# Christovis/astrild

Hardware: AMD Instinct MI355X
Metric: particles/sec CIC+3D-FFT P(k) on 1024^3 grid (higher is better)
Workload: dtype f32

## Files before the change

### astrild_amd/csrc/fft_tile.hip

```cpp
#include "ast_common.h"
#include "paint_tile_geom.h"
#include <algorithm>
#include <cmath>
#include <cstring>
#include <mutex>
#include <vector>

namespace {

__device__ constexpr float kCos32[16] = {
    1.0f, 0.9807852804032304f, 0.9238795325112867f, 0.8314696123025452f, 0.7071067811865476f,
    0.5555702330196023f, 0.38268343236508984f, 0.19509032201612833f, 0.0f, -0.1950903220161282f,
    -0.3826834323650897f, -0.555570233019602f, -0.7071067811865475f, -0.8314696123025453f,
    -0.9238795325112867f, -0.9807852804032304f};
__device__ constexpr float kSin32[16] = {
    0.0f, 0.19509032201612825f, 0.3826834323650898f, 0.5555702330196022f, 0.7071067811865475f,
    0.8314696123025452f, 0.9238795325112867f, 0.9807852804032304f, 1.0f, 0.9807852804032304f,
    0.9238795325112867f, 0.8314696123025455f, 0.7071067811865476f, 0.5555702330196022f,
    0.3826834323650899f, 0.1950903220161286f};

#ifndef FFT_NT
#define FFT_NT 3
#endif
typedef float f2v __attribute__((ext_vector_type(2)));
template <bool NT>
__device__ inline float2 ld_stream(const float2* p) {
    if (NT && (FFT_NT & 1)) { const f2v v = __builtin_nontemporal_load(reinterpret_cast<const f2v*>(p)); return make_float2(v.x, v.y); }
    return *p;
}
template <bool NT>
__device__ inline void st_stream(float2* p, float2 v) {
    if (NT && (FFT_NT & 2)) __builtin_nontemporal_store(f2v{v.x, v.y}, reinterpret_cast<f2v*>(p));
    else *p = v;
}
typedef float cf2 __attribute__((ext_vector_type(2)));
__device__ inline cf2 to_cf(float2 a) { return cf2{a.x, a.y}; }
__device__ inline float2 from_cf(cf2 a) { return make_float2(a.x, a.y); }
__device__ inline cf2 cmul_cf(cf2 a, cf2 w) {
    return __builtin_elementwise_fma(a.yy, cf2{-w.y, w.x}, a.xx * w);
}
__device__ inline float2 cmul(float2 a, float2 w) { return from_cf(cmul_cf(to_cf(a), to_cf(w))); }

constexpr int bitrev(int v, int bits) {
    int r = 0;
    for (int i = 0; i < bits; ++i) r |= ((v >> i) & 1) << (bits - 1 - i);
    return r;
}
constexpr int ilog2(int v) { return v <= 1 ? 0 : 1 + ilog2(v / 2); }

template <int R>
__device__ inline void fft_reg(float2 (&vv)[R]) {
    cf2 v[R];
#pragma unroll
    for (int i = 0; i < R; ++i) v[i] = to_cf(vv[i]);
#pragma unroll
    for (int h = R / 2; h >= 1; h /= 2) {
#pragma unroll
        for (int blk = 0; blk < R; blk += 2 * h) {
#pragma unroll
            for (int j = 0; j < h; ++j) {
                const cf2 a = v[blk + j], b = v[blk + j + h];
                v[blk + j] = a + b;
                const cf2 d = a - b;
                const int t = j * (16 / h);
                if (t == 0) v[blk + j + h] = d;
                else if (t == 8) v[blk + j + h] = d.yx * cf2{1.0f, -1.0f};
                else v[blk + j + h] = cmul_cf(d, cf2{kCos32[t], -kSin32[t]});
            }
        }
    }
#pragma unroll
    for (int i = 0; i < R; ++i) vv[i] = from_cf(v[i]);
}

__device__ inline int tile_isqrt(int v) {
    return (int)__builtin_amdgcn_sqrtf((float)v + 0.5f);
}

__global__ void tile_isqrt_table_kernel(int* out, int count) {
    for (int v = blockIdx.x * blockDim.x + threadIdx.x; v < count; v += gridDim.x * blockDim.x) out[v] = tile_isqrt(v);
}

struct ShellMask { const float2* src; long long lo2, hi2; int ky0 = 0; int pass = 0;
                   size_t src_elem_stride = 0, src_batch_stride = 0; };

constexpr int SHELL_BATCH = 8;
#ifndef C2C_XCD_MODE
#define C2C_XCD_MODE 2
#endif
struct ShellBatch { int count = 0; float2* work[SHELL_BATCH]; long long lo2[SHELL_BATCH], hi2[SHELL_BATCH]; };
struct C2RBatch { int count = 0; const float2* in[SHELL_BATCH]; float* out[SHELL_BATCH]; int kmax[SHELL_BATCH]; };

struct DiscEntry { int offb; unsigned S, cumS, lohi; };
struct PackDst { float2* out = nullptr; unsigned c1_log2 = 0; unsigned nbatch = 0; float2* self_out = nullptr; unsigned self_part = ~0u; unsigned pitch = 0;
                 const DiscEntry* disc = nullptr; const unsigned short* gk = nullptr; unsigned part = 0;
                 unsigned xmajor = 0; };

template <int R1, int R2, int C, bool POWER, bool INV = false, int PACK = 0>
__global__ void __launch_bounds__(C * (R1 > R2 ? R1 : R2))
__attribute__((amdgpu_waves_per_eu((POWER || C > 16) && R1 * R2 >= 1024 ? 4 : 1, (POWER || C > 16) && R1 * R2 >= 1024 ? 4 : 8)))
strided_c2c_kernel(float2* __restrict__ data, const float2* __restrict__ tw_g, size_t elem_stride,
                   size_t ncols, size_t batch_stride, unsigned tiles_per_batch, float scale,
                   double* __restrict__ partial, const unsigned* __restrict__ edge_fall, ShellMask mask = ShellMask{nullptr, 0, 0},
                   PackDst pack = PackDst{}, ShellBatch sb = ShellBatch{}) {
    constexpr int N = R1 * R2;
    constexpr int NT = C * (R1 > R2 ? R1 : R2);
    constexpr int NB = N / 2 - 1;
    constexpr bool SPLIT = (POWER || C > 16) && R1 == R2 && N * C * sizeof(float2) > 64 * 1024;
    constexpr int YN = SPLIT ? N / 2 : N;
    extern __shared__ float2 lds[];
    float2* Y = lds;
    float2* tw = lds + YN * C;
    double* shell = reinterpret_cast<double*>(lds + YN * C + N);
    unsigned tile = blockIdx.x % tiles_per_batch, b = blockIdx.x / tiles_per_batch;
#if C2C_XCD_MODE
    if ((INV || C2C_XCD_MODE == 2) && (gridDim.x / tiles_per_batch) % 8u == 0u) {
        const unsigned xcd = blockIdx.x & 7u, slot = blockIdx.x >> 3;
        b = (slot / tiles_per_batch) * 8u + xcd;
        tile = slot % tiles_per_batch;
    }
#endif
    const size_t c0 = (size_t)tile * C;
    if (INV && sb.count > 0) {
        data = sb.work[blockIdx.y];
        mask.lo2 = sb.lo2[blockIdx.y];
        mask.hi2 = sb.hi2[blockIdx.y];
    }
    if (INV && mask.hi2 > 0) {
        const long long kb = (long long)((int)b > N / 2 ? (int)b - N : (int)b);
        const long long r2 = (long long)(c0 * c0) + (mask.pass == 0 ? kb * kb : 0);
        if (r2 >= mask.hi2) return;
    }
    const float2* disc_base = nullptr;
    unsigned disc_S = 0;
    int disc_ky = 0;
    if (!INV && POWER && pack.disc != nullptr) {
        const unsigned subb = b % R1, gk = pack.gk[pack.part * (pack.nbatch / R1) + b / R1];
        const DiscEntry e = pack.disc[(size_t)tile * R2 + gk];
        const unsigned lo = e.lohi & 255u, hi = (e.lohi >> 8) & 255u;
        if (subb - lo >= hi - lo) {
            for (int i = threadIdx.x; i < NB; i += NT) partial[((size_t)b * tiles_per_batch + tile) * NB + i] = 0.0;
            return;
        }
        disc_ky = (int)(gk * R1 + subb);
        if (pack.xmajor) {
            disc_base = data + ((long long)e.offb + (long long)(subb * 16u)) * (long long)pack.xmajor;
            disc_S = 16u;
        } else {
            disc_base = data + ((long long)e.offb + (long long)(subb * 16u));
            disc_S = e.S;
        }
    } else if (!INV && POWER && mask.hi2 > 0) {
        const long long kyi = (long long)b + mask.ky0, ky = kyi > N / 2 ? kyi - N : kyi;
        if (ky * ky + (long long)(c0 * c0) > mask.hi2) {
            for (int i = threadIdx.x; i < NB; i += NT) partial[((size_t)b * tiles_per_batch + tile) * NB + i] = 0.0;
            return;
        }
    }
    for (int i = threadIdx.x; i < N; i += NT) tw[i] = tw_g[i];
    if (POWER)
        for (int i = threadIdx.x; i <= NB; i += NT) shell[i] = 0.0;
    const int c = threadIdx.x % C, sub = threadIdx.x / C;
    const bool col_ok = (unsigned)c0 + (unsigned)c < (unsigned)ncols;
    float2 u[R2];
    {
        const bool task1 = sub < R2;
        float2 v[R1];
        const bool own = INV && mask.src != nullptr && mask.src_elem_stride != 0;
        size_t es_in = own ? mask.src_elem_stride : elem_stride;
        const float2* ubase = (INV && mask.src ? mask.src : data) + (size_t)b * (own ? mask.src_batch_stride : batch_stride);
        const int lsub = task1 ? sub : R2 - 1;
        uint32_t voff = (uint32_t)lsub * (uint32_t)es_in + min((uint32_t)c0 + (uint32_t)c, (uint32_t)ncols - 1u);
        if (POWER && !INV && disc_base != nullptr) {
            es_in = disc_S;
            ubase = disc_base;
            voff = (uint32_t)lsub * disc_S + (uint32_t)c;
        }
        if (INV && mask.hi2 > 0 && mask.pass == 1) {
            const long long c02 = (long long)(c0 * c0);
#pragma unroll
            for (int n1 = 0; n1 < R1; ++n1) {
                const int row = n1 * R2 + lsub;
                const long long ky = row > N / 2 ? row - N : row;
                v[n1] = make_float2(0.f, 0.f);
                if (ky * ky + c02 < mask.hi2) v[n1] = (ubase + (size_t)(n1 * R2) * es_in)[voff];
            }
        } else if (INV && mask.hi2 > 0) {
            const long long kyb = (long long)((int)b > N / 2 ? (int)b - N : (int)b);
            const long long r2yz = kyb * kyb + (long long)(c0 * c0);
#pragma unroll
            for (int n1 = 0; n1 < R1; ++n1) {
                const int lo = n1 * R2, hi = lo + R2 - 1;
                const long long kxmin = hi <= N / 2 ? lo : (lo >= N / 2 ? N - hi : 0);
                v[n1] = make_float2(0.f, 0.f);
                if (kxmin * kxmin + r2yz < mask.hi2) v[n1] = (ubase + (size_t)(n1 * R2) * es_in)[voff];
            }
        } else {
#pragma unroll
            for (int n1 = 0; n1 < R1; ++n1) v[n1] = ld_stream<(!INV && N >= 1024)>(ubase + (size_t)(n1 * R2) * es_in + voff);
        }
        if (INV) {
            if (mask.hi2 > 0 && mask.pass == 0) {
                const long long kz = (long long)min(c0 + c, ncols - 1), ky = (long long)((int)b > N / 2 ? (int)b - N : (int)b);
                const long long m2yz = ky * ky + kz * kz;
#pragma unroll
                for (int n1 = 0; n1 < R1; ++n1) {
                    const int row = n1 * R2 + lsub;
                    const long long kx = row > N / 2 ? row - N : row, m2 = kx * kx + m2yz;
                    if (m2 < mask.lo2 || m2 >= mask.hi2) v[n1] = make_float2(0.f, 0.f);
                }
            }
#pragma unroll
            for (int n1 = 0; n1 < R1; ++n1) v[n1].y = -v[n1].y;
        }
        fft_reg<R1>(v);
        __syncthreads();
        if (!SPLIT) {
            if (task1) {
#pragma unroll
                for (int k1 = 0; k1 < R1; ++k1) {
                    float2 y = v[bitrev(k1, ilog2(R1))];
                    if (k1 != 0) y = cmul(y, tw[sub * k1]);
                    Y[(sub * R1 + k1) * C + c] = y;
                }
            }
            __syncthreads();
            if (sub < R1) {
#pragma unroll
                for (int n2 = 0; n2 < R2; ++n2) u[n2] = Y[(n2 * R1 + sub) * C + c];
            }
        } else {
            constexpr int H = R2 / 2;
#pragma unroll
            for (int half = 0; half < 2; ++half) {
                if (sub / H == half) {
#pragma unroll
                    for (int k1 = 0; k1 < R1; ++k1) {
                        float2 y = v[bitrev(k1, ilog2(R1))];
                        if (k1 != 0) y = cmul(y, tw[sub * k1]);
                        Y[((sub - half * H) * R1 + k1) * C + c] = y;
                    }
                }
                __syncthreads();
#pragma unroll
                for (int nh = 0; nh < H; ++nh) u[half * H + nh] = Y[(nh * R1 + sub) * C + c];
                if (half == 0) __syncthreads();
            }
        }
    }
    if (sub < R1) {
        fft_reg<R2>(u);
        int tid_s = (int)threadIdx.x;
        if (C > 16) asm volatile("" : "+v"(tid_s));
        const int cs = C > 16 ? tid_s % C : c;
        const bool ok_s = C > 16 ? (unsigned)c0 + (unsigned)cs < (unsigned)ncols : col_ok;
        if (PACK == 2 && !POWER) {
            static_assert(PACK != 2 || C == 16, "the disc layout's tiles are 16 columns");
            const int4 ev = reinterpret_cast<const int4*>(pack.disc + (size_t)tile * R2)[threadIdx.x % R2];
#pragma unroll
            for (int k2 = 0; k2 < R2; ++k2) {
                float2 x = u[bitrev(k2, ilog2(R2))];
                x.x *= scale;
                x.y *= scale;
                const int offb = __builtin_amdgcn_readlane(ev.x, k2);
                const unsigned S = (unsigned)__builtin_amdgcn_readlane(ev.y, k2), cumS = (unsigned)__builtin_amdgcn_readlane(ev.z, k2);
                const unsigned lohi = (unsigned)__builtin_amdgcn_readlane(ev.w, k2);
                const unsigned lo = lohi & 255u, hi = (lohi >> 8) & 255u, part = lohi >> 16;
                if (pack.xmajor) {
                    float2* const ub = pack.self_out + ((long long)offb * (long long)pack.xmajor + (long long)(b * 16u));
                    if ((unsigned)sub - lo < hi - lo)
                        st_stream<(N >= 1024)>(ub + ((uint32_t)sub * 16u * pack.xmajor + (uint32_t)(threadIdx.x & 15u)), x);
                    continue;
                }
                float2* const ub = (part == pack.self_part ? pack.self_out : pack.out + (size_t)pack.nbatch * cumS)
                                   + ((size_t)b * S + (long long)offb);
                if ((unsigned)sub - lo < hi - lo) st_stream<(N >= 1024)>(ub + threadIdx.x, x);
            }
        } else if (ok_s && !POWER) {
            float2* const base = data + (size_t)b * batch_stride + c0 + cs;
            const int room = (!INV && mask.hi2 > 0) ? (int)mask.hi2 - (int)(c0 * c0) : 0x7fffffff;
            const int wsub0 = __builtin_amdgcn_readfirstlane((int)threadIdx.x) / C, wsub1 = wsub0 + 64 / C - 1;
#pragma unroll
            for (int k2 = 0; k2 < R2; ++k2) {
                float2 x = u[bitrev(k2, ilog2(R2))];
                x.x *= scale;
                x.y *= INV ? -scale : scale;
                if (!INV) {
                    const int aky = R1 * k2 >= N / 2 ? N - (wsub1 + R1 * k2) : wsub0 + R1 * k2;
                    if (aky * aky > room) continue;
                }
                if (PACK) {
                    const unsigned part = (unsigned)(R1 * k2) >> pack.c1_log2, r0 = (unsigned)(R1 * k2) & ((1u << pack.c1_log2) - 1u);
                    float2* const ub = part == pack.self_part
                        ? pack.self_out + ((((size_t)b) << pack.c1_log2) + r0) * pack.pitch
                        : pack.out + ((((size_t)part * pack.nbatch + b) << pack.c1_log2) + r0) * pack.pitch;
                    st_stream<(N >= 1024)>(ub + ((uint32_t)sub * pack.pitch + (uint32_t)c0 + (uint32_t)cs), x);
                } else {
                    st_stream<(!INV && N >= 1024)>(base + (size_t)(sub + R1 * k2) * elem_stride, x);
                }
            }
        }
    }
    int tid_e = (int)threadIdx.x;
    asm volatile("" : "+v"(tid_e));
    if (POWER && (unsigned)c0 + (unsigned)(tid_e % C) < (unsigned)ncols && sub < R1) {
        unsigned fallmask = 0;
        const int kyi = disc_base != nullptr ? disc_ky : (int)b + mask.ky0;
        if (edge_fall) fallmask = edge_fall[((size_t)(disc_base != nullptr ? (unsigned)disc_ky : b) * tiles_per_batch + tile) * NT + threadIdx.x];
        const int kz = (int)c0 + tid_e % C;
        const int ky = kyi > N / 2 ? kyi - N : kyi;
        const int m2yz = ky * ky + kz * kz;
        const float w = (kz > 0 && kz < N / 2) ? 2.0f : 1.0f;
#pragma unroll
        for (int k2 = 0; k2 < R2; ++k2) {
            const float2 x = u[bitrev(k2, ilog2(R2))];
            const int row = sub + R1 * k2;
            const int kx = row > N / 2 ? row - N : row;
            int sh = tile_isqrt(kx * kx + m2yz);
            sh -= (int)((fallmask >> k2) & 1u);
            if (sh >= 1 && sh <= NB) atomicAdd(&shell[sh], (double)(fmaf(x.x, x.x, x.y * x.y) * w));
        }
    }
    if (POWER) {
        __syncthreads();
        const double s2 = (double)scale * (double)scale;
        for (int i = threadIdx.x; i < NB; i += NT) partial[((size_t)b * tiles_per_batch + tile) * NB + i] = shell[i + 1] * s2;
    }
}

constexpr int REDUCE_ROWS = 1024;
__global__ void __launch_bounds__(256)
shell_partials_stage1_kernel(const double* __restrict__ partial, size_t nwg, int nb, double* __restrict__ partial2) {
    const size_t per = (nwg + REDUCE_ROWS - 1) / REDUCE_ROWS;
    const size_t g0 = (size_t)blockIdx.x * per, g1 = g0 + per < nwg ? g0 + per : nwg;
    for (int bin = threadIdx.x; bin < nb; bin += 256) {
        double acc = 0.0;
#pragma unroll 8
        for (size_t g = g0; g < g1; ++g) acc += partial[g * nb + bin];
        partial2[(size_t)blockIdx.x * nb + bin] = acc;
    }
}
__global__ void __launch_bounds__(256)
shell_partials_stage2_kernel(const double* __restrict__ partial2, int nb, double pnorm, int first_bin,
                             double* __restrict__ psum) {
    __shared__ double part[32][8];
    const int b8 = threadIdx.x & 7, grp = threadIdx.x >> 3;
    const int bin = blockIdx.x * 8 + b8;
    double acc = 0.0;
    if (bin < nb) {
#pragma unroll 8
        for (int r = grp; r < REDUCE_ROWS; r += 32) acc += partial2[(size_t)r * nb + bin];
    }
    part[grp][b8] = acc;
    __syncthreads();
    if (grp == 0 && bin < nb && bin >= first_bin) {
        double t = 0.0;
        for (int k = 0; k < 32; ++k) t += part[k][b8];
        psum[bin] += pnorm * t;
    }
}

constexpr int MLOW_FWD = 5, MBOX_FWD = MLOW_FWD + 1;
__device__ constexpr double kC16f[16] = {1.0, 0.92387953251128674, 0.70710678118654752, 0.38268343236508977, 0.0,
                                         -0.38268343236508977, -0.70710678118654752, -0.92387953251128674, -1.0,
                                         -0.92387953251128674, -0.70710678118654752, -0.38268343236508977, 0.0,
                                         0.38268343236508977, 0.70710678118654752, 0.92387953251128674};
__device__ constexpr double kS16f[16] = {0.0, -0.38268343236508977, -0.70710678118654752, -0.92387953251128674, -1.0,
                                         -0.92387953251128674, -0.70710678118654752, -0.38268343236508977, 0.0,
                                         0.38268343236508977, 0.70710678118654752, 0.92387953251128674, 1.0,
                                         0.92387953251128674, 0.70710678118654752, 0.38268343236508977};

struct SlabFold { int xb0 = 0, ntx = 0, row_lo = 0, row_hi = 0; bool ranges = false; };

template <int R1, int R2, int C, int FOLDW, bool LOWK = false>
__global__ void __launch_bounds__(C * R2)
__attribute__((amdgpu_waves_per_eu(LOWK ? 4 : 1, LOWK ? 4 : 8)))
rows_r2c_kernel(const float* __restrict__ in, float2* __restrict__ out, const float2* __restrict__ tw_g,
                size_t nrows, size_t in_pitch, size_t out_pitch, float scale, float mean,
                const float* __restrict__ rec, const double2* __restrict__ lowk_lane = nullptr,
                double* __restrict__ lowz = nullptr, SlabFold sf = SlabFold{}) {
    constexpr int M = R1 * R2, N = 2 * M;
    constexpr int NT = C * R2;
    constexpr int R2P = R2 + 1;
    constexpr int MP = M + 1;
    extern __shared__ float2 lds[];
    float2* Y = lds;
    float2* tw = lds + C * (R1 * R2P > MP ? R1 * R2P : MP);
    for (int i = threadIdx.x; i < N; i += NT) tw[i] = tw_g[i];

    const size_t row0 = (size_t)blockIdx.x * C;
    const int n2 = threadIdx.x % R2, r = threadIdx.x / R2;
    {
        const float2* zin = reinterpret_cast<const float2*>(in + min(row0 + r, nrows - 1) * in_pitch);
        float2 v[R1];
#pragma unroll
        for (int n1 = 0; n1 < R1; ++n1) v[n1] = ld_stream<(N >= 1024)>(zin + n1 * R2 + n2);
        if (FOLDW != 0) {
            constexpr int W = FOLDW != 0 ? FOLDW : 2;
            const int ng = (int)(2 * M);
            const size_t row = min(row0 + r, nrows - 1);
            const float* src[3];
            int ns;
            if (sf.ntx == 0) {
                const int xb = sf.xb0 + (int)(row / ng), trow = xb / ast::TX;
                ns = !sf.ranges || (trow >= sf.row_lo && trow < sf.row_hi)
                         ? ast::halo_sources<float, W>(rec, xb, (int)(row % ng), ng, ng / ast::TX, ng / ast::TY, src) : 0;
            } else {
                const int xb = sf.xb0 + (int)(row / ng), trow = xb / ast::TX;
                ns = trow >= sf.row_lo && trow < sf.row_hi
                         ? ast::halo_sources<float, W>(rec, xb, (int)(row % ng), ng, sf.ntx, ng / ast::TY, src, false) : 0;
            }
            if (ns > 0) {
                float2 h[R1];
#pragma unroll
                for (int n1 = 0; n1 < R1; ++n1) h[n1] = reinterpret_cast<const float2*>(src[0])[n1 * R2 + n2];
                if (ns > 1) {
#pragma unroll
                    for (int n1 = 0; n1 < R1; ++n1) {
                        const float2 t = reinterpret_cast<const float2*>(src[1])[n1 * R2 + n2];
                        h[n1].x += t.x;
                        h[n1].y += t.y;
                    }
                }
                if (ns > 2) {
#pragma unroll
                    for (int n1 = 0; n1 < R1; ++n1) {
                        const float2 t = reinterpret_cast<const float2*>(src[2])[n1 * R2 + n2];
                        h[n1].x += t.x;
                        h[n1].y += t.y;
                    }
                }
#pragma unroll
                for (int n1 = 0; n1 < R1; ++n1) {
                    v[n1].x += h[n1].x;
                    v[n1].y += h[n1].y;
                }
            }
        }
        if (LOWK) {
            static_assert(!LOWK || ((R1 == 16 || R1 == 8) && (R2 == 32 || R2 == 16) && MBOX_FWD == 6), "R1-th roots from the 16th-root table; 32 or 16 lanes per row");
            double acc[14];
#pragma unroll
            for (int e = 0; e < 14; ++e) acc[e] = 0.0;
#pragma unroll
            for (int p = 0; p < 2; ++p) {
                double f[R1];
#pragma unroll
                for (int n1 = 0; n1 < R1; ++n1) f[n1] = (double)(p ? v[n1].y : v[n1].x);
#pragma unroll
                for (int kz = 0; kz <= MBOX_FWD; ++kz) {
                    double tr = 0.0, ti = 0.0;
#pragma unroll
                    for (int n1 = 0; n1 < R1; ++n1) {
                        const int rr = ((kz * n1) % R1) * (16 / R1);
                        if (rr == 0) tr += f[n1];
                        else if (rr == 4) ti -= f[n1];
                        else if (rr == 8) tr -= f[n1];
                        else if (rr == 12) ti += f[n1];
                        else { tr = fma(f[n1], kC16f[rr], tr); ti = fma(f[n1], kS16f[rr], ti); }
                    }
                    const double2 a = lowk_lane[(n2 * (MBOX_FWD + 1) + kz) * 2 + p];
                    acc[2 * kz] = fma(a.x, tr, fma(-a.y, ti, acc[2 * kz]));
                    acc[2 * kz + 1] = fma(a.x, ti, fma(a.y, tr, acc[2 * kz + 1]));
                }
            }
            const int lane = threadIdx.x & 63;
            auto level = [&](auto count_tag, int mask) {
                constexpr int COUNT = decltype(count_tag)::value;
                const bool upper = (lane & mask) != 0;
#pragma unroll
                for (int i = 0; i < COUNT / 2; ++i) {
                    const double keep = upper ? acc[i + COUNT / 2] : acc[i];
                    const double send = upper ? acc[i] : acc[i + COUNT / 2];
                    acc[i] = keep + __shfl_xor(send, mask, 64);
                }
            };
            constexpr int TOP = R2 / 2;
            level(std::integral_constant<int, 14>{}, TOP);
            acc[7] = 0.0;
            level(std::integral_constant<int, 8>{}, TOP / 2);
            level(std::integral_constant<int, 4>{}, TOP / 4);
            level(std::integral_constant<int, 2>{}, TOP / 8);
            if (R2 == 32) acc[0] += __shfl_xor(acc[0], 1, 64);
            constexpr int SH = R2 == 32 ? 1 : 0;
            const int sel = lane >> SH;
            const int sub = ((sel >> 2) & 1) * 4 + ((sel >> 1) & 1) * 2 + (sel & 1);
            if ((R2 == 16 || (lane & 1) == 0) && sub < 7 && row0 + r < nrows)
                lowz[(row0 + r) * (size_t)(2 * (MBOX_FWD + 1)) + ((sel >> 3) & 1) * 7 + sub] = acc[0];
        }
#pragma unroll
        for (int n1 = 0; n1 < R1; ++n1) {
            v[n1].x -= mean;
            v[n1].y -= mean;
        }
        fft_reg<R1>(v);
        __syncthreads();
#pragma unroll
        for (int k1 = 0; k1 < R1; ++k1) {
            float2 y = v[bitrev(k1, ilog2(R1))];
            if (k1 != 0) y = cmul(y, tw[2 * n2 * k1]);
            Y[(r * R1 + k1) * R2P + n2] = y;
        }
    }
    __syncthreads();
    float2 u[R2];
    const int k1 = threadIdx.x % R1, r2 = threadIdx.x / R1;
    const bool task2 = r2 < C;
    if (task2) {
#pragma unroll
        for (int j = 0; j < R2; ++j) u[j] = Y[(r2 * R1 + k1) * R2P + j];
        fft_reg<R2>(u);
    }
    __syncthreads();
    if (task2) {
#pragma unroll
        for (int k2 = 0; k2 < R2; ++k2) Y[r2 * MP + k1 + R1 * k2] = u[bitrev(k2, ilog2(R2))];
    }
    __syncthreads();
    for (int i = threadIdx.x; i < C * (M / 2 + 1); i += NT) {
        const int rr = i / (M / 2 + 1), k = i % (M / 2 + 1);
        if (row0 + rr >= nrows) continue;
        const float2 zk = Y[rr * MP + k];
        const float2 zm = Y[rr * MP + ((M - k) & (M - 1))];
        float2* orow = out + (row0 + rr) * out_pitch;
        if (k == 0) {
            orow[0] = make_float2((zk.x + zk.y) * scale, 0.f);
            orow[M] = make_float2((zk.x - zk.y) * scale, 0.f);
            continue;
        }
        const float2 e = make_float2(0.5f * (zk.x + zm.x), 0.5f * (zk.y - zm.y));
        const float2 o = make_float2(0.5f * (zk.x - zm.x), 0.5f * (zk.y + zm.y));
        const float2 w = tw[k];
        const float2 t = cmul(o, w);
        st_stream<(N >= 1024)>(orow + k, make_float2((e.x + t.y) * scale, (e.y - t.x) * scale));
        st_stream<(N >= 1024)>(orow + M - k, make_float2((e.x - t.y) * scale, (-e.y - t.x) * scale));
    }
}

template <int R1, int R2, int C>
__global__ void __launch_bounds__(C * R2)
rows_c2r_kernel(const float2* __restrict__ in, float* __restrict__ out, const float2* __restrict__ tw_g,
                size_t nrows, size_t in_pitch, size_t out_pitch, float scale, int kmax, C2RBatch cb = C2RBatch{}) {
    if (cb.count > 0) { in = cb.in[blockIdx.y]; out = cb.out[blockIdx.y]; kmax = cb.kmax[blockIdx.y]; }
    constexpr int M = R1 * R2, N = 2 * M;
    constexpr int NT = C * R2;
    constexpr int R2P = R2 + 1;
    constexpr int MP = M + 1;
    extern __shared__ float2 lds[];
    float2* Y = lds;
    float2* tw = lds + C * (R1 * R2P > MP ? R1 * R2P : MP);
    for (int i = threadIdx.x; i < N; i += NT) tw[i] = tw_g[i];
    const size_t row0 = (size_t)blockIdx.x * C;
    {
        const int rr = threadIdx.x / R2, q = threadIdx.x % R2;
        const float2* src = in + min(row0 + rr, nrows - 1) * in_pitch;
        float2 tmp[R1 + 1];
#pragma unroll
        for (int i = 0; i <= R1; ++i) {
            tmp[i] = make_float2(0.f, 0.f);
            if (i * R2 < kmax) tmp[i] = src[min(q + R2 * i, M)];
        }
#pragma unroll
        for (int i = 0; i <= R1; ++i) {
            const int k = q + R2 * i;
            if (k <= M) Y[rr * MP + k] = k < kmax ? tmp[i] : make_float2(0.f, 0.f);
        }
    }
    __syncthreads();
    const int n2 = threadIdx.x % R2, r = threadIdx.x / R2;
    float2 v[R1];
#pragma unroll
    for (int n1 = 0; n1 < R1; ++n1) {
        const int k = n1 * R2 + n2;
        const float2 xk = Y[r * MP + k], xm = Y[r * MP + M - k];
        const float2 e = make_float2(0.5f * (xk.x + xm.x), 0.5f * (xk.y - xm.y));
        const float2 d = make_float2(0.5f * (xk.x - xm.x), 0.5f * (xk.y + xm.y));
        const float2 w = tw[k];
        const float2 t = make_float2(d.x * w.x + d.y * w.y, d.y * w.x - d.x * w.y);
        v[n1] = make_float2(e.x - t.y, -(e.y + t.x));
    }
    __syncthreads();
    fft_reg<R1>(v);
#pragma unroll
    for (int k1 = 0; k1 < R1; ++k1) {
        float2 y = v[bitrev(k1, ilog2(R1))];
        if (k1 != 0) y = cmul(y, tw[2 * n2 * k1]);
        Y[(r * R1 + k1) * R2P + n2] = y;
    }
    __syncthreads();
    float2 u[R2];
    const int k1 = threadIdx.x % R1, r2 = threadIdx.x / R1;
    const bool task2 = r2 < C;
    if (task2) {
#pragma unroll
        for (int j = 0; j < R2; ++j) u[j] = Y[(r2 * R1 + k1) * R2P + j];
        fft_reg<R2>(u);
    }
    __syncthreads();
    if (task2) {
#pragma unroll
        for (int k2 = 0; k2 < R2; ++k2) Y[r2 * MP + k1 + R1 * k2] = u[bitrev(k2, ilog2(R2))];
    }
    __syncthreads();
    const float s2 = 2.0f * scale;
#ifndef C2R_ST
#define C2R_ST 2
#endif
    if (C2R_ST) {
        typedef float f4v __attribute__((ext_vector_type(4)));
        for (int i = threadIdx.x; i < C * (M / 2); i += NT) {
            const int rr = i / (M / 2), j = (i % (M / 2)) * 2;
            if (row0 + rr >= nrows) continue;
            const float2 z0 = Y[rr * MP + j], z1 = Y[rr * MP + j + 1];
            const f4v o = {z0.x * s2, -z0.y * s2, z1.x * s2, -z1.y * s2};
            f4v* dst = reinterpret_cast<f4v*>(out + (row0 + rr) * out_pitch) + j / 2;
            if (C2R_ST == 2) __builtin_nontemporal_store(o, dst); else *dst = o;
        }
        return;
    }
    for (int i = threadIdx.x; i < C * M; i += NT) {
        const int rr = i / M, j = i % M;
        if (row0 + rr >= nrows) continue;
        const float2 z = Y[rr * MP + j];
// ... 77 lines not shown
            v[n1] = make_float2(e.x - tt.y, -(e.y + tt.x));
        }
        __syncthreads();
        fft_reg<R1>(v);
#pragma unroll
        for (int k1 = 0; k1 < R1; ++k1) {
            float2 y = v[bitrev(k1, ilog2(R1))];
            if (k1 != 0) y = cmul(y, tw[2 * n2 * k1]);
            Y[(r * R1 + k1) * R2P + n2] = y;
        }
        __syncthreads();
        float2 u[R2];
        const int k1 = threadIdx.x % R1, r2 = threadIdx.x / R1;
        const bool task2 = r2 < C;
        if (task2) {
#pragma unroll
            for (int j = 0; j < R2; ++j) u[j] = Y[(r2 * R1 + k1) * R2P + j];
            fft_reg<R2>(u);
        }
        __syncthreads();
        if (task2) {
#pragma unroll
            for (int k2 = 0; k2 < R2; ++k2) {
                const float2 zz = u[bitrev(k2, ilog2(R2))];
                Y[r2 * MP + k1 + R1 * k2] = make_float2(zz.x, -zz.y);
            }
        }
        __syncthreads();
        if (PREFETCH && pos + gridDim.x < nrows) fetch(pos + gridDim.x);
#ifndef TRI_FUSE_ABLATE
#define TRI_FUSE_ABLATE 0
#endif
        if (worker && !(TRI_FUSE_ABLATE & 1)) {
            const float* f = reinterpret_cast<const float*>(Y);
            float s0 = 0.f, s1 = 0.f;
            if (wave_pairs) {
#pragma unroll 4
                for (int c = c_lo; c < c_hi; c += 2) {
                    const float2 x = *reinterpret_cast<const float2*>(f + ia + c), y = *reinterpret_cast<const float2*>(f + ic + c);
                    s0 = fmaf(x.x * x.x, y.x, s0);
                    s1 = fmaf(x.y * x.y, y.y, s1);
                }
            } else {
#pragma unroll 4
                for (int c = c_lo; c < c_hi; c += 2) {
                    const float2 x = *reinterpret_cast<const float2*>(f + ia + c), y = *reinterpret_cast<const float2*>(f + ib + c);
                    const float2 z = *reinterpret_cast<const float2*>(f + ic + c);
                    s0 = fmaf(x.x * y.x, z.x, s0);
                    s1 = fmaf(x.y * y.y, z.y, s1);
                }
            }
            acc += (double)s0 + (double)s1;
        }
        __syncthreads();
    }
    partial[(size_t)blockIdx.x * NT + threadIdx.x] = worker ? acc : 0.0;
}

__global__ void __launch_bounds__(256)
triangles_reduce_kernel(const double* __restrict__ partial, int nblocks, int nthreads, int ntri, int parts, double factor,
                        double* __restrict__ out) {
    const int t = blockIdx.x;
    double acc = 0.0;
    for (int i = threadIdx.x; i < nblocks * parts; i += 256) {
        const int blk = i / parts, part = i % parts;
        acc += partial[(size_t)blk * nthreads + part * ntri + t];
    }
    for (int o = 32; o > 0; o >>= 1) acc += __shfl_xor(acc, o, 64);
    __shared__ double w[4];
    if ((threadIdx.x & 63) == 0) w[threadIdx.x >> 6] = acc;
    __syncthreads();
    if (threadIdx.x == 0) out[t] = factor * ((w[0] + w[1]) + (w[2] + w[3]));
}

constexpr int MLOW = 5;
constexpr int MBOX = MLOW + 1;
__device__ constexpr double kC32o[16] = {0.98078528040323044, 0.83146961230254524, 0.55557023301960222, 0.19509032201612827,
                                         -0.19509032201612827, -0.55557023301960222, -0.83146961230254524, -0.98078528040323044,
                                         -0.98078528040323044, -0.83146961230254524, -0.55557023301960222, -0.19509032201612827,
                                         0.19509032201612827, 0.55557023301960222, 0.83146961230254524, 0.98078528040323044};
__device__ constexpr double kS32o[16] = {-0.19509032201612827, -0.55557023301960222, -0.83146961230254524, -0.98078528040323044,
                                         -0.98078528040323044, -0.83146961230254524, -0.55557023301960222, -0.19509032201612827,
                                         0.19509032201612827, 0.55557023301960222, 0.83146961230254524, 0.98078528040323044,
                                         0.98078528040323044, 0.83146961230254524, 0.55557023301960222, 0.19509032201612827};
__device__ constexpr double kC16[16] = {1.0, 0.92387953251128674, 0.70710678118654752, 0.38268343236508977, 0.0,
                                        -0.38268343236508977, -0.70710678118654752, -0.92387953251128674, -1.0,
                                        -0.92387953251128674, -0.70710678118654752, -0.38268343236508977, 0.0,
                                        0.38268343236508977, 0.70710678118654752, 0.92387953251128674};
__device__ constexpr double kS16[16] = {0.0, -0.38268343236508977, -0.70710678118654752, -0.92387953251128674, -1.0,
                                        -0.92387953251128674, -0.70710678118654752, -0.38268343236508977, 0.0,
                                        0.38268343236508977, 0.70710678118654752, 0.92387953251128674, 1.0,
                                        0.92387953251128674, 0.70710678118654752, 0.38268343236508977};

template <int COUNT>
__device__ inline void reduce_level(double (&v)[28], int lane, int mask) {
    const bool upper = (lane & mask) != 0;
#pragma unroll
    for (int i = 0; i < COUNT / 2; ++i) {
        const double keep = upper ? v[i + COUNT / 2] : v[i];
        const double send = upper ? v[i] : v[i + COUNT / 2];
        v[i] = keep + __shfl_xor(send, mask, 64);
    }
}

template <int NJ, int FOLDW>
__global__ void __launch_bounds__(256)
lowk_z_kernel(const float* __restrict__ grid, const float* __restrict__ rec, int n, size_t nrows, double2* __restrict__ out) {
    static_assert(MBOX == 6, "the reduction below is laid out for 2 rows x 7 kz x (re, im) = 28 sums");
    const int lane = threadIdx.x & 63;
    double twc[MBOX + 1], tws[MBOX + 1];
#pragma unroll
    for (int kz = 0; kz <= MBOX; ++kz) sincospi(-2.0 * (double)((kz * lane) % n) / (double)n, &tws[kz], &twc[kz]);
    const size_t npairs = nrows / 2, nwaves = (size_t)gridDim.x * 4;
    for (size_t pair = (size_t)blockIdx.x * 4 + (threadIdx.x >> 6); pair < npairs; pair += nwaves) {
        double v[28];
#pragma unroll
        for (int rr = 0; rr < 2; ++rr) {
            const size_t row = 2 * pair + rr;
            const float* in = grid + row * (size_t)n;
            float fr[NJ];
#pragma unroll
            for (int j = 0; j < NJ; ++j) fr[j] = in[lane + 64 * j];
            if (FOLDW != 0) {
                constexpr int W = FOLDW != 0 ? FOLDW : 2;
                const float* src[3];
                const int ns = ast::halo_sources<float, W>(rec, (int)(row / n), (int)(row % n), n, n / ast::TX, n / ast::TY, src);
                if (ns > 0) {
                    float h[NJ];
#pragma unroll
                    for (int j = 0; j < NJ; ++j) h[j] = src[0][lane + 64 * j];
                    if (ns > 1) {
#pragma unroll
                        for (int j = 0; j < NJ; ++j) h[j] += src[1][lane + 64 * j];
                    }
                    if (ns > 2) {
#pragma unroll
                        for (int j = 0; j < NJ; ++j) h[j] += src[2][lane + 64 * j];
                    }
#pragma unroll
                    for (int j = 0; j < NJ; ++j) fr[j] += h[j];
                }
            }
            double f[NJ];
#pragma unroll
            for (int j = 0; j < NJ; ++j) f[j] = (double)fr[j];
#pragma unroll
            for (int kz = 0; kz <= MBOX; ++kz) {
                double re = 0.0, im = 0.0;
#pragma unroll
                for (int j = 0; j < NJ; ++j) {
                    if (NJ <= 16) {
                        constexpr int step = NJ <= 16 ? 16 / NJ : 1;
                        const int r = ((kz * j) % NJ) * step;
                        if (r == 0) re += f[j];
                        else if (r == 4) im -= f[j];
                        else if (r == 8) re -= f[j];
                        else if (r == 12) im += f[j];
                        else { re += f[j] * kC16[r]; im += f[j] * kS16[r]; }
                    } else {
                        const int r = (kz * j) % 32;
                        if (r == 0) re += f[j];
                        else if (r == 8) im -= f[j];
                        else if (r == 16) re -= f[j];
                        else if (r == 24) im += f[j];
                        else if (r % 2 == 0) { re += f[j] * kC16[r / 2]; im += f[j] * kS16[r / 2]; }
                        else { re += f[j] * kC32o[r / 2]; im += f[j] * kS32o[r / 2]; }
                    }
                }
                v[rr * 14 + 2 * kz] = re * twc[kz] - im * tws[kz];
                v[rr * 14 + 2 * kz + 1] = re * tws[kz] + im * twc[kz];
            }
        }
        reduce_level<28>(v, lane, 32);
        reduce_level<14>(v, lane, 16);
        v[7] = 0.0;
        reduce_level<8>(v, lane, 8);
        reduce_level<4>(v, lane, 4);
        reduce_level<2>(v, lane, 2);
        v[0] += __shfl_xor(v[0], 1, 64);
        const int sub = ((lane >> 3) & 1) * 4 + ((lane >> 2) & 1) * 2 + ((lane >> 1) & 1);
        if ((lane & 1) == 0 && sub < 7) {
            const int e = ((lane >> 5) & 1) * 14 + ((lane >> 4) & 1) * 7 + sub;
            reinterpret_cast<double*>(out)[(2 * pair + e / 14) * (size_t)(2 * (MBOX + 1)) + e % 14] = v[0];
        }
    }
}

constexpr int LOWK_XPARTS = 64;
__global__ void __launch_bounds__(256)
lowk_axis_kernel(const double2* __restrict__ in, int n, int nt, int t0, int inner, double2* __restrict__ out) {
    extern __shared__ double2 tw[];
    for (int t = threadIdx.x; t < n; t += 256) {
        double sn, cs;
        sincospi(-2.0 * (double)t / (double)n, &sn, &cs);
        tw[t] = make_double2(cs, sn);
    }
    __syncthreads();
    const size_t outer = blockIdx.x;
    const int nparts = gridDim.y, part = blockIdx.y;
    const int per = (nt + nparts - 1) / nparts, ta = part * per, tb = min(nt, ta + per);
    const int nout = (2 * MBOX + 1) * inner;
    if (nout <= 128) {
        __shared__ double2 part_sum[256];
        const int groups = 256 / nout, o = threadIdx.x % nout, gq = threadIdx.x / nout;
        double re = 0.0, im = 0.0, re2 = 0.0, im2 = 0.0;
        if (gq < groups) {
            const int k = o / inner - MBOX, i = o % inner;
            int t = ta + gq;
            for (; t + groups < tb; t += 2 * groups) {
                const double2 v = in[(outer * nt + t) * inner + i], v2 = in[(outer * nt + t + groups) * inner + i];
                const double2 w = tw[(unsigned)(k * (t0 + t)) & (unsigned)(n - 1)];
                const double2 w2 = tw[(unsigned)(k * (t0 + t + groups)) & (unsigned)(n - 1)];
                re += v.x * w.x - v.y * w.y;
                im += v.x * w.y + v.y * w.x;
                re2 += v2.x * w2.x - v2.y * w2.y;
                im2 += v2.x * w2.y + v2.y * w2.x;
            }
            if (t < tb) {
                const double2 v = in[(outer * nt + t) * inner + i];
                const double2 w = tw[(unsigned)(k * (t0 + t)) & (unsigned)(n - 1)];
                re += v.x * w.x - v.y * w.y;
                im += v.x * w.y + v.y * w.x;
            }
        }
        part_sum[threadIdx.x] = make_double2(re + re2, im + im2);
        __syncthreads();
        if (gq == 0) {
            double sr = 0.0, si = 0.0;
            for (int q = 0; q < groups; ++q) { sr += part_sum[q * nout + o].x; si += part_sum[q * nout + o].y; }
            const int k = o / inner - MBOX, i = o % inner;
            out[((outer * nparts + part) * (2 * MBOX + 1) + k + MBOX) * inner + i] = make_double2(sr, si);
        }
        return;
    }
    for (int o = threadIdx.x; o < nout; o += 256) {
        const int k = o / inner - MBOX, i = o % inner;
        double re[4] = {0.0, 0.0, 0.0, 0.0}, im[4] = {0.0, 0.0, 0.0, 0.0};
        for (int tq = ta; tq < tb; tq += 4) {
#pragma unroll
            for (int q = 0; q < 4; ++q) {
                const int t = min(tq + q, tb - 1);
                const double2 v = in[(outer * nt + t) * inner + i];
                const double2 w = tw[(unsigned)(k * (t0 + t)) & (unsigned)(n - 1)];
                if (tq + q < tb) {
                    re[q] += v.x * w.x - v.y * w.y;
                    im[q] += v.x * w.y + v.y * w.x;
                }
            }
        }
        out[((outer * nparts + part) * (2 * MBOX + 1) + k + MBOX) * inner + i] =
            make_double2((re[0] + re[1]) + (re[2] + re[3]), (im[0] + im[1]) + (im[2] + im[3]));
    }
}

__global__ void __launch_bounds__(256)
lowk_parts_reduce_kernel(const double2* __restrict__ in, int nparts, int count, int accumulate, double2* __restrict__ acc) {
    const int i = blockIdx.x * 256 + threadIdx.x;
    if (i >= count) return;
    double re = accumulate ? acc[i].x : 0.0, im = accumulate ? acc[i].y : 0.0;
    for (int p = 0; p < nparts; ++p) {
        re += in[(size_t)p * count + i].x;
        im += in[(size_t)p * count + i].y;
    }
    acc[i] = make_double2(re, im);
}

__global__ void __launch_bounds__(256)
lowk_shell_kernel(const double2* __restrict__ modes, double pnorm, double kf_rule, double* __restrict__ sums) {
    constexpr int NM = (2 * MBOX + 1) * (2 * MBOX + 1) * (MBOX + 1);
    __shared__ double val[NM];
    __shared__ signed char sh[NM];
    for (int i = threadIdx.x; i < NM; i += 256) {
        const int c = i % (MBOX + 1), b = (i / (MBOX + 1)) % (2 * MBOX + 1) - MBOX, a = i / ((MBOX + 1) * (2 * MBOX + 1)) - MBOX;
        const int m2 = a * a + b * b + c * c;
        int r = (int)sqrt((double)m2);
        while (r * r > m2) --r;
        while ((r + 1) * (r + 1) <= m2) ++r;
        if (kf_rule != 0.0 && r * r == m2 && r > 0) r = ast::float64_edge_norm(r, a, b, c, kf_rule);
        const double2 v = modes[i];
        sh[i] = (signed char)(r - 1 < MLOW ? r - 1 : -1);
        val[i] = (c > 0 ? 2.0 : 1.0) * (v.x * v.x + v.y * v.y);
    }
    __syncthreads();
    if ((int)threadIdx.x < MLOW) {
        double acc = 0.0;
        for (int i = 0; i < NM; ++i)
            if (sh[i] == (int)threadIdx.x) acc += val[i];
        sums[threadIdx.x] = acc * pnorm;
    }
}

__global__ void lowk_patch_kernel(const double* __restrict__ sums, int count, double* __restrict__ psum) {
    if ((int)threadIdx.x < count) psum[threadIdx.x] += sums[threadIdx.x];
}

template <int R1, int R2, int C>
__global__ void edge_fall_kernel(unsigned* __restrict__ out, unsigned tiles_per_batch, int ncols, double kf) {
    constexpr int N = R1 * R2;
    const unsigned tile = blockIdx.x % tiles_per_batch, b = blockIdx.x / tiles_per_batch;
    const int c = threadIdx.x % C, sub = threadIdx.x / C;
    const int kz = (int)(tile * C + c), ky = (int)b > N / 2 ? (int)b - N : (int)b;
    unsigned word = 0;
    if (sub < R1 && kz < ncols) {
        for (int k2 = 0; k2 < R2; ++k2) {
            const int row = sub + R1 * k2, kx = row > N / 2 ? row - N : row;
            const int m2 = kx * kx + ky * ky + kz * kz;
            int r = (int)sqrt((double)m2);
            while (r * r > m2) --r;
            while ((r + 1) * (r + 1) <= m2) ++r;
            if (r * r == m2 && r > 0 && ast::float64_edge_norm(r, kx, ky, kz, kf) != r) word |= 1u << k2;
        }
    }
    out[(size_t)blockIdx.x * blockDim.x + threadIdx.x] = word;
}

struct EdgeFallCache {
    std::mutex m;
    struct Entry { int dev; size_t n; double boxsize; unsigned* words; };
    std::vector<Entry> tabs;
    const unsigned* get(size_t n, double boxsize, hipStream_t s) {
        std::lock_guard<std::mutex> lock(m);
        int dev = 0;
        if (hipGetDevice(&dev) != hipSuccess) return nullptr;
        for (auto& t : tabs) if (t.dev == dev && t.n == n && t.boxsize == boxsize) return t.words;
        const size_t nz = n / 2 + 1, tiles = (nz + 15) / 16;
        const unsigned nt = n == 256 ? 256 : 512;
        unsigned* d = nullptr;
        if (hipMalloc(&d, n * tiles * nt * sizeof(unsigned)) != hipSuccess) return nullptr;
        const double kf = 2.0 * M_PI / boxsize;
        const unsigned blocks = (unsigned)(n * tiles);
        if (n == 1024) edge_fall_kernel<32, 32, 16><<<blocks, nt, 0, s>>>(d, (unsigned)tiles, (int)nz, kf);
        else if (n == 512) edge_fall_kernel<16, 32, 16><<<blocks, nt, 0, s>>>(d, (unsigned)tiles, (int)nz, kf);
        else edge_fall_kernel<16, 16, 16><<<blocks, nt, 0, s>>>(d, (unsigned)tiles, (int)nz, kf);
        if (hipGetLastError() != hipSuccess) return nullptr;
        if (tabs.size() >= 4) { (void)hipFree(tabs.front().words); tabs.erase(tabs.begin()); }
        tabs.push_back({dev, n, boxsize, d});
        return d;
    }
} g_edge;

struct TwiddleCache {
    std::mutex m;
    std::vector<std::pair<std::pair<int, int>, float2*>> tabs;
    float2* get(int n) {
        std::lock_guard<std::mutex> lock(m);
        int dev = 0;
        if (hipGetDevice(&dev) != hipSuccess) return nullptr;
        for (auto& t : tabs) if (t.first.first == dev && t.first.second == n) return t.second;
        std::vector<float2> h(n);
        for (int i = 0; i < n; ++i) {
            const double a = -2.0 * M_PI * (double)i / (double)n;
            h[i] = make_float2((float)std::cos(a), (float)std::sin(a));
        }
        float2* d = nullptr;
        if (hipMalloc(&d, n * sizeof(float2)) != hipSuccess) return nullptr;
        if (hipMemcpy(d, h.data(), n * sizeof(float2), hipMemcpyHostToDevice) != hipSuccess) return nullptr;
        tabs.push_back({{dev, n}, d});
        return d;
    }
} g_tw;

template <int R1, int R2, int C, bool POWER>
int launch_c2c(float2* data, const float2* tw, size_t elem_stride, size_t ncols, size_t batch, size_t batch_stride,
               float scale, double* partial, hipStream_t s, const unsigned* edge_fall = nullptr, int ky0 = 0, long long prune2 = 0,
               PackDst disc = PackDst{}) {
    constexpr int N = R1 * R2, NT = C * (R1 > R2 ? R1 : R2);
    constexpr bool SPLIT = (POWER || C > 16) && R1 == R2 && N * C * sizeof(float2) > 64 * 1024;
    const size_t lds = (size_t)((SPLIT ? N / 2 : N) * C + N) * sizeof(float2) + (POWER ? (N / 2) * sizeof(double) : 0);
    static ast::PerDeviceOnce attr_once;
    if (attr_once.need()) {
        AST_CHECK_HIP(hipFuncSetAttribute(reinterpret_cast<const void*>(&strided_c2c_kernel<R1, R2, C, POWER>),
                                          hipFuncAttributeMaxDynamicSharedMemorySize, (int)lds));
        attr_once.mark();
    }
    const size_t tiles = (ncols + C - 1) / C;
    AST_CHECK_ARG(tiles * batch < 0x7fffffffull);
    AST_CHECK_ARG((size_t)(R2 - 1) * elem_stride + ncols < (1ull << 29));
    strided_c2c_kernel<R1, R2, C, POWER><<<(unsigned)(tiles * batch), NT, lds, s>>>(data, tw, elem_stride, ncols,
                                                                                   batch_stride, (unsigned)tiles, scale,
                                                                                   partial, edge_fall, ShellMask{nullptr, 0, prune2, ky0}, disc);
    AST_CHECK_LAUNCH();
    return AST_OK;
}

template <int R1, int R2, int C>
int launch_c2c_inv(float2* data, const float2* tw, size_t elem_stride, size_t ncols, size_t batch, size_t batch_stride,
                   float scale, ShellMask mask, hipStream_t s, ShellBatch sb = ShellBatch{}) {
    constexpr int N = R1 * R2, NT = C * (R1 > R2 ? R1 : R2);
    const size_t lds = (size_t)(N * C + N) * sizeof(float2);
    static ast::PerDeviceOnce attr_once;
    if (attr_once.need()) {
        AST_CHECK_HIP(hipFuncSetAttribute(reinterpret_cast<const void*>(&strided_c2c_kernel<R1, R2, C, false, true>),
                                          hipFuncAttributeMaxDynamicSharedMemorySize, (int)lds));
        attr_once.mark();
    }
    const size_t tiles = (ncols + C - 1) / C;
    AST_CHECK_ARG(tiles * batch < 0x7fffffffull);
    AST_CHECK_ARG((size_t)(R2 - 1) * elem_stride + ncols < (1ull << 29));
    strided_c2c_kernel<R1, R2, C, false, true><<<dim3((unsigned)(tiles * batch), (unsigned)(sb.count > 0 ? sb.count : 1)), NT, lds, s>>>(
        data, tw, elem_stride, ncols, batch_stride, (unsigned)tiles, scale, nullptr, nullptr, mask, PackDst{}, sb);
    AST_CHECK_LAUNCH();
    return AST_OK;
}

template <int R1, int R2, int C, int PACKM = 1>
int launch_c2c_pack(float2* data, const float2* tw, size_t elem_stride, size_t ncols, size_t batch, size_t batch_stride,
                    float scale, PackDst pack, hipStream_t s) {
    constexpr int N = R1 * R2, NT = C * (R1 > R2 ? R1 : R2);
    constexpr bool SPLIT = C > 16 && R1 == R2 && N * C * sizeof(float2) > 64 * 1024;
    const size_t lds = (size_t)((SPLIT ? N / 2 : N) * C + N) * sizeof(float2);
    static ast::PerDeviceOnce attr_once;
    if (attr_once.need()) {
        AST_CHECK_HIP(hipFuncSetAttribute(reinterpret_cast<const void*>(&strided_c2c_kernel<R1, R2, C, false, false, PACKM>),
                                          hipFuncAttributeMaxDynamicSharedMemorySize, (int)lds));
        attr_once.mark();
    }
    const size_t tiles = (ncols + C - 1) / C;
    AST_CHECK_ARG(tiles * batch < 0x7fffffffull);
    AST_CHECK_ARG((size_t)(R2 - 1) * elem_stride + ncols < (1ull << 29));
    strided_c2c_kernel<R1, R2, C, false, false, PACKM><<<(unsigned)(tiles * batch), NT, lds, s>>>(
        data, tw, elem_stride, ncols, batch_stride, (unsigned)tiles, scale, nullptr, nullptr, ShellMask{nullptr, 0, 0}, pack);
    AST_CHECK_LAUNCH();
    return AST_OK;
}

int dispatch_c2c_inv(size_t n, float2* d, const float2* tw, size_t elem_stride, size_t ncols, size_t batch, size_t batch_stride,
                     float scale, ShellMask mask, hipStream_t s, ShellBatch sb = ShellBatch{}) {
    if (n == 1024) return launch_c2c_inv<32, 32, 16>(d, tw, elem_stride, ncols, batch, batch_stride, scale, mask, s, sb);
    if (n == 512) return launch_c2c_inv<16, 32, 16>(d, tw, elem_stride, ncols, batch, batch_stride, scale, mask, s, sb);
    return launch_c2c_inv<16, 16, 16>(d, tw, elem_stride, ncols, batch, batch_stride, scale, mask, s, sb);
}

template <bool POWER>
int dispatch_c2c(size_t n, float2* d, const float2* tw, size_t elem_stride, size_t ncols, size_t batch,
                 size_t batch_stride, float scale, double* partial, hipStream_t s, const unsigned* edge_fall = nullptr, int ky0 = 0,
                 long long prune2 = 0, PackDst disc = PackDst{}) {
#ifndef FWD_C
#define FWD_C 32
#endif
    if constexpr (!POWER) { if (n == 1024) return launch_c2c<32, 32, FWD_C, false>(d, tw, elem_stride, ncols, batch, batch_stride, scale, partial, s, edge_fall, ky0, prune2); }
    if (n == 1024) return launch_c2c<32, 32, 16, POWER>(d, tw, elem_stride, ncols, batch, batch_stride, scale, partial, s, edge_fall, ky0, prune2, disc);
    if (n == 512) return launch_c2c<16, 32, 16, POWER>(d, tw, elem_stride, ncols, batch, batch_stride, scale, partial, s, edge_fall, ky0, prune2, disc);
    return launch_c2c<16, 16, 16, POWER>(d, tw, elem_stride, ncols, batch, batch_stride, scale, partial, s, edge_fall, ky0, prune2, disc);
}

template <int R1, int R2, int C, int FOLDW = 0, bool LOWK = false>
int launch_r2c(const float* in, float2* out, const float2* tw, size_t nrows, size_t in_pitch, size_t out_pitch,
               float scale, float mean, hipStream_t s, const float* rec = nullptr, const double2* lowk_lane = nullptr,
               double* lowz = nullptr, SlabFold sf = SlabFold{}) {
    constexpr int M = R1 * R2, N = 2 * M, NT = C * R2;
    constexpr int BUF = C * (R1 * (R2 + 1) > M + 1 ? R1 * (R2 + 1) : M + 1);
    const size_t lds = (size_t)(BUF + N) * sizeof(float2);
    static ast::PerDeviceOnce attr_once;
    if (attr_once.need()) {
        AST_CHECK_HIP(hipFuncSetAttribute(reinterpret_cast<const void*>(&rows_r2c_kernel<R1, R2, C, FOLDW, LOWK>),
                                          hipFuncAttributeMaxDynamicSharedMemorySize, (int)lds));
        attr_once.mark();
    }
    const size_t blocks = (nrows + C - 1) / C;
    AST_CHECK_ARG(blocks < 0x7fffffffull);
    rows_r2c_kernel<R1, R2, C, FOLDW, LOWK><<<(unsigned)blocks, NT, lds, s>>>(in, out, tw, nrows, in_pitch, out_pitch, scale, mean, rec,
                                                                             lowk_lane, lowz, sf);
    AST_CHECK_LAUNCH();
    return AST_OK;
}

template <int R1, int R2, int C>
int launch_c2r(const float2* in, float* out, const float2* tw, size_t nrows, size_t in_pitch, size_t out_pitch, float scale,
               int kmax, hipStream_t s, C2RBatch cb = C2RBatch{}) {
    constexpr int M = R1 * R2, N = 2 * M, NT = C * R2;
    constexpr int BUF = C * (R1 * (R2 + 1) > M + 1 ? R1 * (R2 + 1) : M + 1);
    const size_t lds = (size_t)(BUF + N) * sizeof(float2);
    static ast::PerDeviceOnce attr_once;
    if (attr_once.need()) {
        AST_CHECK_HIP(hipFuncSetAttribute(reinterpret_cast<const void*>(&rows_c2r_kernel<R1, R2, C>),
                                          hipFuncAttributeMaxDynamicSharedMemorySize, (int)lds));
        attr_once.mark();
    }
    const size_t blocks = (nrows + C - 1) / C;
    AST_CHECK_ARG(blocks < 0x7fffffffull);
    rows_c2r_kernel<R1, R2, C><<<dim3((unsigned)blocks, (unsigned)(cb.count > 0 ? cb.count : 1)), NT, lds, s>>>(in, out, tw, nrows, in_pitch, out_pitch,
                                                                                                        scale, kmax, cb);
    AST_CHECK_LAUNCH();
    return AST_OK;
}

constexpr int tile_r1(size_t n) { return n == 1024 ? 32 : 16; }
struct DiscLayout {
    size_t n = 0;
    int parts = 0, r1 = 0;
    unsigned nblk = 0, tiles = 0;
    std::vector<unsigned> S, cumS;
    std::vector<unsigned short> gk;
    std::vector<unsigned char> part_of;
    std::vector<DiscEntry> tab;
    struct Dev { int dev; DiscEntry* tab; unsigned short* gk; };
    std::vector<Dev> devs;
    unsigned total() const { return cumS.back() + S.back(); }
};

static bool disc_row_in(size_t n, int row, unsigned tile) {
    const long long ky = row > (int)(n / 2) ? row - (long long)n : row, kz0 = 16ll * tile, h = (long long)(n / 2);
    return ky * ky + kz0 * kz0 <= h * h;
}

static void disc_build(DiscLayout& L, size_t n, int parts) {
    L.n = n; L.parts = parts; L.r1 = tile_r1(n);
    L.nblk = (unsigned)(n / L.r1); L.tiles = (unsigned)((n / 2 + 1 + 15) / 16);
    const unsigned nb = L.nblk / parts;
    std::vector<unsigned> area(L.nblk, 0);
    for (unsigned k = 0; k < L.nblk; ++k)
        for (int sub = 0; sub < L.r1; ++sub)
            for (unsigned t = 0; t < L.tiles; ++t) area[k] += disc_row_in(n, (int)(k * L.r1 + sub), t) ? 1u : 0u;
    std::vector<unsigned> order(L.nblk);
    for (unsigned k = 0; k < L.nblk; ++k) order[k] = k;
    std::stable_sort(order.begin(), order.end(), [&](unsigned a, unsigned b) { return area[a] > area[b]; });
    std::vector<unsigned long long> sum(parts, 0);
    std::vector<unsigned> cnt(parts, 0);
    L.part_of.assign(L.nblk, 0);
    for (unsigned k : order) {
        int best = -1;
        for (int r = 0; r < parts; ++r)
            if (cnt[r] < nb && (best < 0 || sum[r] < sum[best])) best = r;
        L.part_of[k] = (unsigned char)best;
        sum[best] += area[k];
        ++cnt[best];
    }
    L.gk.clear();
    for (int r = 0; r < parts; ++r)
        for (unsigned k = 0; k < L.nblk; ++k)
            if (L.part_of[k] == r) L.gk.push_back((unsigned short)k);
    L.tab.assign((size_t)L.tiles * L.nblk, DiscEntry{0, 0, 0, 0});
    L.S.assign(parts, 0);
    L.cumS.assign(parts, 0);
    for (int r = 0; r < parts; ++r) {
        unsigned rows = 0;
        for (unsigned t = 0; t < L.tiles; ++t)
            for (unsigned j = 0; j < nb; ++j) {
                const unsigned k = L.gk[(size_t)r * nb + j];
                int lo = -1, hi = -1;
                for (int sub = 0; sub < L.r1; ++sub)
                    if (disc_row_in(n, (int)(k * L.r1 + sub), t)) { if (lo < 0) lo = sub; hi = sub + 1; }
                DiscEntry& e = L.tab[(size_t)t * L.nblk + k];
                if (lo < 0) { e.lohi = (unsigned)r << 16; continue; }
                e.offb = 16 * ((int)rows - lo);
                e.lohi = (unsigned)lo | (unsigned)hi << 8 | (unsigned)r << 16;
                rows += (unsigned)(hi - lo);
            }
        L.S[r] = 16 * rows;
    }
    for (int r = 1; r < parts; ++r) L.cumS[r] = L.cumS[r - 1] + L.S[r - 1];
    for (auto& e : L.tab) { const unsigned r = e.lohi >> 16; e.S = L.S[r]; e.cumS = L.cumS[r]; }
}

struct DiscCache {
    std::mutex m;
    std::vector<DiscLayout*> all;
    const DiscLayout* get(size_t n, int parts, bool device, const DiscLayout::Dev** dv) {
        std::lock_guard<std::mutex> lock(m);
        DiscLayout* L = nullptr;
        for (auto* x : all) if (x->n == n && x->parts == parts) L = x;
        if (!L) { L = new DiscLayout; disc_build(*L, n, parts); all.push_back(L); }
        if (!device) return L;
        int dev = 0;
        if (hipGetDevice(&dev) != hipSuccess) return nullptr;
        for (auto& d : L->devs) if (d.dev == dev) { *dv = &d; return L; }
        DiscLayout::Dev d{dev, nullptr, nullptr};
        if (hipMalloc(&d.tab, L->tab.size() * sizeof(DiscEntry)) != hipSuccess) return nullptr;
        if (hipMalloc(&d.gk, L->gk.size() * sizeof(unsigned short)) != hipSuccess) return nullptr;
        if (hipMemcpy(d.tab, L->tab.data(), L->tab.size() * sizeof(DiscEntry), hipMemcpyHostToDevice) != hipSuccess) return nullptr;
        if (hipMemcpy(d.gk, L->gk.data(), L->gk.size() * sizeof(unsigned short), hipMemcpyHostToDevice) != hipSuccess) return nullptr;
        L->devs.reserve(64);
        L->devs.push_back(d);
        *dv = &L->devs.back();
        return L;
    }
} g_disc;

static bool disc_geometry_ok(size_t n, int parts) {
    return (n == 256 || n == 512 || n == 1024) && parts >= 1 && parts <= 256 && (n / tile_r1(n)) % (size_t)parts == 0;
}

}

extern "C" int ast_fft_tile_supported(int dtype, size_t n) {
    return dtype == AST_F32 && (n == 256 || n == 512 || n == 1024) ? 1 : 0;
}

extern "C" int ast_fft_tile_c2c(void* data, int dtype, size_t n, size_t elem_stride, size_t ncols, size_t batch,
                                size_t batch_stride, double scale, void* stream) {
    AST_CHECK_ARG(data != nullptr && ncols >= 1 && batch >= 1 && elem_stride >= ncols);
    AST_CHECK_ARG(ast_fft_tile_supported(dtype, n));
    const float2* tw = g_tw.get((int)n);
    if (!tw) { ast::set_error("ast_fft_tile_c2c: twiddle table allocation failed"); return AST_ERR_HIP; }
    hipStream_t s = ast::as_stream(stream);
    AST_PROF("fft_tile.c2c", s);
    return dispatch_c2c<false>(n, (float2*)data, tw, elem_stride, ncols, batch, batch_stride, (float)scale, nullptr, s);
}

extern "C" int ast_fft_tile_c2c_packed(const void* planes, void* packed, int dtype, size_t n, size_t ncols, size_t pitch,
                                       size_t nplanes, int parts, int self_part, void* self_out, double scale, void* stream) {
    AST_CHECK_ARG(planes != nullptr && planes != packed && planes != self_out && ncols >= 1 && nplanes >= 1 && pitch >= ncols);
    AST_CHECK_ARG((self_out == nullptr) || (self_part >= 0 && self_part < parts));
    AST_CHECK_ARG(packed != nullptr || (self_out != nullptr && parts == 1));
    AST_CHECK_ARG(ast_fft_tile_supported(dtype, n));
    AST_CHECK_ARG(parts >= 1 && (parts & (parts - 1)) == 0 && n % (size_t)parts == 0);
    AST_CHECK_ARG(n / (size_t)parts >= (n == 1024 ? 32u : 16u));
    AST_CHECK_ARG(pitch < (1u << 24));
    const float2* tw = g_tw.get((int)n);
    if (!tw) { ast::set_error("ast_fft_tile_c2c_packed: twiddle table allocation failed"); return AST_ERR_HIP; }
    hipStream_t s = ast::as_stream(stream);
    PackDst pack;
    pack.out = (float2*)packed;
// ... 594 lines not shown
```

Measured before the change: 83.36 billion.

## Pair ±kx power terms across lanes to halve shell atomic adds

In the power-spectrum pass, threads are remapped so that each sub handles a k1 whose mirror frequency (−kx) sits in the partner lane (lane ^ 16). The two power values are combined with a ds_swizzle before one double atomicAdd per |kx| shell, so each thread issues about half as many LDS atomics. The edge-fall table is recomputed to match the new indexing. This adds swizzle traffic and special cases for k1=0 and R1/2, and the subtle index mapping carries some risk of correctness bugs.

New measurement: 84.19 billion (median of 6 runs). Within noise of the previous version (+1.0%).

```diff
diff --git a/astrild_amd/csrc/fft_tile.hip b/astrild_amd/csrc/fft_tile.hip
--- a/astrild_amd/csrc/fft_tile.hip
+++ b/astrild_amd/csrc/fft_tile.hip
@@ -75,6 +75,11 @@
 
 __device__ inline int tile_isqrt(int v) {
     return (int)__builtin_amdgcn_sqrtf((float)v + 0.5f);
+}
+
+template <int R1>
+__host__ __device__ constexpr int power_k1(int sub) {
+    return (sub & 1) == 0 ? sub >> 1 : ((sub >> 1) == 0 ? R1 / 2 : R1 - (sub >> 1));
 }
 
 __global__ void tile_isqrt_table_kernel(int* out, int count) {
@@ -215,6 +220,9 @@
         }
         fft_reg<R1>(v);
         __syncthreads();
+        int tid_k = (int)threadIdx.x;
+        if (POWER) asm volatile("" : "+v"(tid_k));
+        const int k1t = POWER ? power_k1<R1>(tid_k / C) : sub;
         if (!SPLIT) {
             if (task1) {
 #pragma unroll
@@ -227,7 +235,7 @@
             __syncthreads();
             if (sub < R1) {
 #pragma unroll
-                for (int n2 = 0; n2 < R2; ++n2) u[n2] = Y[(n2 * R1 + sub) * C + c];
+                for (int n2 = 0; n2 < R2; ++n2) u[n2] = Y[(n2 * R1 + k1t) * C + c];
             }
         } else {
             constexpr int H = R2 / 2;
@@ -243,7 +251,7 @@
                 }
                 __syncthreads();
 #pragma unroll
-                for (int nh = 0; nh < H; ++nh) u[half * H + nh] = Y[(nh * R1 + sub) * C + c];
+                for (int nh = 0; nh < H; ++nh) u[half * H + nh] = Y[(nh * R1 + k1t) * C + c];
                 if (half == 0) __syncthreads();
             }
         }
@@ -311,14 +319,26 @@
         const int ky = kyi > N / 2 ? kyi - N : kyi;
         const int m2yz = ky * ky + kz * kz;
         const float w = (kz > 0 && kz < N / 2) ? 2.0f : 1.0f;
+        static_assert(!POWER || C == 16, "the pair partner is lane ^ 16: one 16-column row per sub");
+        const int k1 = power_k1<R1>(sub);
+        float p[R2];
 #pragma unroll
         for (int k2 = 0; k2 < R2; ++k2) {
             const float2 x = u[bitrev(k2, ilog2(R2))];
-            const int row = sub + R1 * k2;
-            const int kx = row > N / 2 ? row - N : row;
+            p[k2] = fmaf(x.x, x.x, x.y * x.y) * w;
+        }
+#pragma unroll
+        for (int i = 0; i < R2 / 2; ++i) {
+            const float other = __int_as_float(__builtin_amdgcn_ds_swizzle(__float_as_int(p[R2 - 1 - i]), 0x401F));
+            const float mirror = k1 == R1 / 2 ? p[R2 - 1 - i] : k1 == 0 ? (i == 0 ? 0.0f : p[(R2 - i) % R2]) : other;
+            const int kx = k1 + R1 * i;
             int sh = tile_isqrt(kx * kx + m2yz);
-            sh -= (int)((fallmask >> k2) & 1u);
-            if (sh >= 1 && sh <= NB) atomicAdd(&shell[sh], (double)(fmaf(x.x, x.x, x.y * x.y) * w));
+            sh -= (int)((fallmask >> i) & 1u);
+            if (sh >= 1 && sh <= NB) atomicAdd(&shell[sh], (double)p[i] + (double)mirror);
+        }
+        if (k1 == 0) {
+            const int sh = tile_isqrt(N / 2 * (N / 2) + m2yz) - (int)((fallmask >> (R2 / 2)) & 1u);
+            if (sh >= 1 && sh <= NB) atomicAdd(&shell[sh], (double)p[R2 / 2]);
         }
     }
     if (POWER) {
@@ -1002,13 +1022,14 @@
     const int kz = (int)(tile * C + c), ky = (int)b > N / 2 ? (int)b - N : (int)b;
     unsigned word = 0;
     if (sub < R1 && kz < ncols) {
-        for (int k2 = 0; k2 < R2; ++k2) {
-            const int row = sub + R1 * k2, kx = row > N / 2 ? row - N : row;
+        const int k1 = power_k1<R1>(sub);
+        for (int i = 0; i < R2 / 2 + (k1 == 0 ? 1 : 0); ++i) {
+            const int kx = k1 + R1 * i;
             const int m2 = kx * kx + ky * ky + kz * kz;
             int r = (int)sqrt((double)m2);
             while (r * r > m2) --r;
             while ((r + 1) * (r + 1) <= m2) ++r;
-            if (r * r == m2 && r > 0 && ast::float64_edge_norm(r, kx, ky, kz, kf) != r) word |= 1u << k2;
+            if (r * r == m2 && r > 0 && ast::float64_edge_norm(r, kx, ky, kz, kf) != r) word |= 1u << i;
         }
     }
     out[(size_t)blockIdx.x * blockDim.x + threadIdx.x] = word;
```
